# darskkaa/NTIRE-2026-Light-Field-Image-Super-Resolution-Challenge---Track-2-Efficiency

Hardware: AMD Instinct MI355X
Metric: 5x5 x4-SR LF patches/sec (32^2->128^2), DistgSSR inference (higher is better)
Workload: dtype f32 (EPI branch stage 1 / 2 and fuse.0: fp32 operands as three exact bf16 terms on the bf16 MFMA pipe, six products, fp32 accumulation -- error against fp64 not above the fp32-MFMA kernels', tests/test_gpu_b3_accuracy.py; 3x3 convs, angular branch, init, head: fp32 MFMA)

## Files before the change

### include/lfsr_hip.h

```cpp
#ifndef LFSR_HIP_H
#define LFSR_HIP_H

#include <stddef.h>
#include <stdint.h>

#ifdef __cplusplus
extern "C" {
#endif

#define LFSR_OK 0
#define LFSR_E_ARG (-1)
#define LFSR_E_WS (-2)

const char* lfsr_version(void);


int lfsr_sai2macpi(const void* in, void* out, int B, int C, int A, int h, int w, int elem_bytes, void* stream);
int lfsr_macpi2sai(const void* in, void* out, int B, int C, int A, int h, int w, int elem_bytes, void* stream);
int lfsr_pixel_shuffle2d(const void* in, void* out, int B, int C, int r, int H, int W, int elem_bytes, void* stream);
int lfsr_pixel_shuffle1d(const void* in, void* out, int B, int C, int f, int H, int W, int elem_bytes, void* stream);
int lfsr_image_extend(const void* in, void* out, int N, int h, int w, int top, int bottom, int left, int right,
                      int elem_bytes, void* stream);
int lfsr_lf_divide(const void* in, void* out, int A, int h0, int w0, int P, int S, int elem_bytes,
                   int* num_u, int* num_v, void* stream);
// ... 24 lines not shown
int lfsr_angconv_fwd(const float* x, int x_stride, int x_choff, const float* w1_packed, const float* w2_packed,
                     float* tmp, float* y, int y_stride, int y_choff, int B, int A, int h, int w, float slope, void* stream);

int lfsr_epiconv_fwd(const float* x, int x_stride, int x_choff, const float* w1_packed, const float* w2_packed,
                     float* tmp, float* y, int y_stride, int y_choff, int B, int A, int h, int w, int vertical,
                     float slope, void* stream);

int lfsr_epiconv_hv_fwd(const float* x, int x_stride, int x_choff, const float* w1_packed, const float* w2_packed,
                        float* tmp, float* y, int y_stride, int choff_h, int choff_v, int B, int A, int h, int w,
                        float slope, void* stream);

int lfsr_distg_branch_tail_fwd(const float* x, int x_stride, int x_choff, const float* spa, int spa_stride, int spa_choff,
                               const float* w_ang0, const float* w_ang2, const float* w_epi0, const float* w_epi2, const float* w_fuse0,
                               float* t_a, float* t_h, float* t_v, float* y, int y_stride, int y_choff, int B, int A, int h, int w, float slope,
                               void* stream);

int lfsr_initconv_fwd(const float* x, const float* w, float* y, int y_stride, int y_choff, int B, int A, int h, int wd,
                      void* stream);

int lfsr_fold_head(const float* w0, const float* b0, const float* w2, float* wf, float* bf, int C, int s, void* stream);
int lfsr_upsample_head_fwd(const float* f, int f_stride, int f_choff, const float* wf, const float* bf,
                           const float* x_lr, float* out, int B, int A, int h, int w, int s, void* stream);

typedef struct lfsr_distgssr lfsr_distgssr;

int lfsr_distgssr_create(lfsr_distgssr** ctx, int A, int scale, int n_group, int n_block, int channels);
void lfsr_distgssr_destroy(lfsr_distgssr* ctx);
size_t lfsr_distgssr_packed_bytes(const lfsr_distgssr* ctx);
int lfsr_distgssr_set_packed(lfsr_distgssr* ctx, void* packed, size_t bytes);
int lfsr_distgssr_load_param(lfsr_distgssr* ctx, const char* key, const float* data, size_t numel, void* stream);
// ... 181 lines not shown
```

### ntire-2026-light-field-image-super-resolution-challenge---track-2-efficiency_amd/capi.py

```python
import ctypes as C
import os

import torch

_HERE = os.path.dirname(os.path.abspath(__file__))
LIB_PATH = os.environ.get("LFSR_HIP_LIB") or os.path.join(_HERE, "liblfsr_hip.so")

c_p = C.c_void_p
c_i = C.c_int
c_f = C.c_float
c_sz = C.c_size_t

SIGNATURES = {
    "lfsr_version": (C.c_char_p, []),
    "lfsr_sai2macpi": (c_i, [c_p, c_p, c_i, c_i, c_i, c_i, c_i, c_i, c_p]),
    "lfsr_macpi2sai": (c_i, [c_p, c_p, c_i, c_i, c_i, c_i, c_i, c_i, c_p]),
    "lfsr_pixel_shuffle2d": (c_i, [c_p, c_p, c_i, c_i, c_i, c_i, c_i, c_i, c_p]),
    "lfsr_pixel_shuffle1d": (c_i, [c_p, c_p, c_i, c_i, c_i, c_i, c_i, c_i, c_p]),
    "lfsr_image_extend": (c_i, [c_p, c_p, c_i, c_i, c_i, c_i, c_i, c_i, c_i, c_i, c_p]),
    "lfsr_lf_divide": (c_i, [c_p, c_p, c_i, c_i, c_i, c_i, c_i, c_i, C.POINTER(c_i), C.POINTER(c_i), c_p]),
    "lfsr_lf_integrate": (c_i, [c_p, c_p, c_i, c_i, c_i, c_i, c_i, c_i, c_i, c_i, c_p]),
    "lfsr_lf_crop_tiles": (c_i, [c_p, c_p, c_i, c_i, c_i, c_i, c_i, c_p]),
    "lfsr_lf_place_tiles": (c_i, [c_p, c_p, c_i, c_i, c_i, c_i, c_i, c_i, c_i, c_i, c_i, c_p]),
    "lfsr_nchw_to_vcl": (c_i, [c_p, c_p, c_i, c_i, c_i, c_i, c_i, c_i, c_i, c_i, c_p]),
    "lfsr_vcl_to_nchw": (c_i, [c_p, c_i, c_i, c_p, c_i, c_i, c_i, c_i, c_i, c_i, c_p]),
    "lfsr_pack_conv_weight": (c_i, [c_p, c_p, c_i, c_i, c_i, c_i, c_i, c_p]),
    "lfsr_packed_weight_floats": (c_sz, [c_i, c_i, c_i]),
    "lfsr_conv3x3_fwd": (c_i, [c_p, c_i, c_i, c_p, c_p, c_i, c_i, c_p, c_i, c_i, c_p, c_i, c_i, c_i, c_i, c_i, c_f, c_p]),
    "lfsr_pointwise_fwd": (c_i, [c_p, c_i, c_i, c_i, c_p, c_p, c_p, c_i, c_i, c_i, c_i, c_f, c_p]),
    "lfsr_angconv_fwd": (c_i, [c_p, c_i, c_i, c_p, c_p, c_p, c_p, c_i, c_i, c_i, c_i, c_i, c_i, c_f, c_p]),
    "lfsr_epiconv_fwd": (c_i, [c_p, c_i, c_i, c_p, c_p, c_p, c_p, c_i, c_i, c_i, c_i, c_i, c_i, c_i, c_f, c_p]),
    "lfsr_epiconv_hv_fwd": (c_i, [c_p, c_i, c_i, c_p, c_p, c_p, c_p, c_i, c_i, c_i, c_i, c_i, c_i, c_i, c_f, c_p]),
    "lfsr_distg_branch_tail_fwd": (c_i, [c_p, c_i, c_i, c_p, c_i, c_i, c_p, c_p, c_p, c_p, c_p, c_p, c_p, c_p, c_p, c_i, c_i, c_i, c_i, c_i, c_i, c_f, c_p]),
    "lfsr_initconv_fwd": (c_i, [c_p, c_p, c_p, c_i, c_i, c_i, c_i, c_i, c_i, c_p]),
    "lfsr_fold_head": (c_i, [c_p, c_p, c_p, c_p, c_p, c_i, c_i, c_p]),
    "lfsr_upsample_head_fwd": (c_i, [c_p, c_i, c_i, c_p, c_p, c_p, c_p, c_i, c_i, c_i, c_i, c_i, c_p]),
    "lfsr_distgssr_begin_batched_load": (c_i, [c_p]),
    "lfsr_distgssr_forward_taps": (c_i, [c_p, c_p, c_p, c_i, c_i, c_i, c_p, c_sz, C.POINTER(c_p), c_p]),
    "lfsr_layernorm_fwd": (c_i, [c_p, c_i, c_i, c_p, c_i, C.c_longlong, C.c_longlong, c_p, c_p, c_p, c_i, c_i, C.c_longlong, c_i, c_f, c_p]),
    "lfsr_conv3x3_n_fwd": (c_i, [c_p, c_i, c_i, c_p, c_p, c_i, c_i, c_i, c_i, c_i, c_i, c_f, c_p]),
    "lfsr_lft_position_fwd": (c_i, [c_p, c_p, c_i, c_i, c_i, c_i, c_p]),
    "lfsr_view_metrics": (c_i, [c_p, c_p, c_p, c_p, c_i, c_i, c_i, c_i, c_p]),
    "lfsr_mask_views": (c_i, [c_p, c_p, c_p, c_f, c_i, c_i, c_i, c_i, c_i, c_p]),
    "lfsr_mask_views_fill": (c_i, [c_p, c_p, c_p, c_p, c_i, c_i, c_i, c_i, c_i, c_p]),
    "lfsr_linear_fwd": (c_i, [c_p, c_i, c_i, c_i, c_p, c_p, c_p, c_i, c_i, c_p, c_i, c_i, C.c_longlong, c_i, c_f, c_p]),
    "lfsr_ycbcr2rgb_views": (c_i, [c_p, c_p, c_p, c_i, c_i, c_i, C.POINTER(C.c_double), C.POINTER(C.c_double), c_p]),
    "lfsr_ffn_fwd": (c_i, [c_p, c_i, c_i, c_p, c_p, c_p, c_i, c_i, c_p, c_i, c_i, C.c_longlong, c_i, c_i, c_i, c_f, c_p]),
# ... 537 lines not shown
    return out


def distg_branch_tail(x, spa, w_ang0, w_ang2, w_epi0, w_epi2, w_fuse0, B, A, h, w, slope):
    lib = load()
    y = torch.empty((x.shape[0], 64), dtype=torch.float32, device=x.device)
    t_a = torch.empty((B * h * w, 16), dtype=torch.float32, device=x.device)
    t_h = torch.empty((B * A * h * w, 32), dtype=torch.float32, device=x.device)
    t_v = torch.empty((B * A * h * w, 32), dtype=torch.float32, device=x.device)
    check(lib.lfsr_distg_branch_tail_fwd(dev_ptr(x), x.shape[1], 0, dev_ptr(spa), spa.shape[1], 0, dev_ptr(w_ang0), dev_ptr(w_ang2), dev_ptr(w_epi0),
                                         dev_ptr(w_epi2), dev_ptr(w_fuse0), dev_ptr(t_a), dev_ptr(t_h), dev_ptr(t_v), dev_ptr(y), 64, 0, B, A, h, w, slope,
                                         stream_ptr()), "distg_branch_tail_fwd")
    return y, t_a, t_h, t_v


def initconv(x, w, A):
    lib = load()
    B, _, Hh, Ww = x.shape
    h, wd = Hh // A, Ww // A
    out = torch.empty((B * A * A * h * wd, 64), dtype=torch.float32, device=x.device)
    check(lib.lfsr_initconv_fwd(dev_ptr(x), dev_ptr(w), dev_ptr(out), 64, 0, B, A, h, wd, stream_ptr()), "initconv_fwd")
    return out


def upsample_head(f, w0, b0, w2, x_lr, A, s):
    lib = load()
    B, _, Hh, Ww = x_lr.shape
    h, w = Hh // A, Ww // A
    wf = torch.empty(s * s * 64, dtype=torch.float32, device=f.device)
    bf = torch.empty(s * s, dtype=torch.float32, device=f.device)
# ... 105 lines not shown
```

### ntire-2026-light-field-image-super-resolution-challenge---track-2-efficiency_amd/csrc/distg_tail.hip

```cpp
#include "lfsr_internal.h"

namespace {

typedef float f32x4t __attribute__((ext_vector_type(4)));
typedef unsigned u32x4t __attribute__((ext_vector_type(4)));

constexpr int DT_WAVES = 8;
constexpr int DT_FPLANE = 64 * 160;
constexpr int DT_FBYTES = 3 * DT_FPLANE * 2;
constexpr int DT_ESLOTS = 3 * 4 * 160;
constexpr int DT_EBYTES = DT_ESLOTS * 16;
constexpr int DT_AFLOATS = 25 * 16 * 16;
constexpr int DT_ABYTES = DT_AFLOATS * 4;
constexpr int DT_CROW = 84;
constexpr int DT_CBYTES = DT_WAVES * 16 * DT_CROW * 4;
constexpr int DT_SMEM = DT_FBYTES + DT_EBYTES + DT_ABYTES + DT_CBYTES;

struct DistgTailArgs {
  const float* S; int s_stride; int s_choff; int s_bytes;
  const float* TA; int ta_bytes;
  const float* TH; const float* TV; int te_bytes;
  const float* WA2;
  const uint4* WE2p;
  const float* WF;
// ... 229 lines not shown
  if (grid > cus[dev]) grid = cus[dev];
  hipLaunchKernelGGL(k_distg_tail, dim3((unsigned)grid), dim3(DT_WAVES * 64), DT_SMEM, st, p);
  LFSR_CHECK_LAUNCH();
  return LFSR_OK;
}

bool lfsr_distg_tail_ok(int A, int h, int w, const float* x, int x_stride, int x_choff, const float* t_h, const float* t_v) {
  if (A != 5 || h <= 0 || w <= 0 || h > 32 || w > 32 || !lfsr_ang_fused_ok(A) || !lfsr_epi_use_b3()) return false;
  const char* rsel = lfsr_sel("LFSR_ROWGEMM");
  const char* asel = lfsr_sel("LFSR_ANG");
  if ((rsel && (rsel[0] == 'f' || rsel[0] == '1')) || lfsr_sel("LFSR_NO_ROWGEMM") || (asel && asel[0] == 'g')) return false;
  if ((x_stride | x_choff) & 3 || x_stride < x_choff + 64 || (((uintptr_t)x | (uintptr_t)t_h | (uintptr_t)t_v) & 15)) return false;
  return true;
}

extern "C" int lfsr_distg_branch_tail_fwd(const float* x, int x_stride, int x_choff, const float* spa, int spa_stride, int spa_choff,
                                          const float* w_ang0, const float* w_ang2, const float* w_epi0, const float* w_epi2, const float* w_fuse0,
                                          float* t_a, float* t_h, float* t_v, float* y, int y_stride, int y_choff, int B, int A, int h, int w, float slope,
                                          void* stream) {
  LfsrOpTimer op_t("distg_tail", B, h * w, lfsr_stream(stream));
  if (!x || !spa || !w_ang0 || !w_ang2 || !w_epi0 || !w_epi2 || !w_fuse0 || !t_a || !t_h || !t_v || !y || B <= 0) return LFSR_E_ARG;
  if (!lfsr_distg_tail_ok(A, h, w, x, x_stride, x_choff, t_h, t_v)) return LFSR_E_ARG;
  if ((spa_stride | spa_choff | y_stride | y_choff) & 3 || spa_stride < spa_choff + 64 || y_stride < y_choff + 64) return LFSR_E_ARG;
  if (((uintptr_t)spa | (uintptr_t)t_a | (uintptr_t)w_ang2 | (uintptr_t)w_epi0 | (uintptr_t)w_epi2 | (uintptr_t)w_fuse0 | (uintptr_t)y) & 15) return LFSR_E_ARG;
  if (!(slope >= 0.f && slope <= 1.f)) return LFSR_E_ARG;
  const long long npix = (long long)B * A * A * h * w;
  if (npix * x_stride * 4 >= (1LL << 31) || npix * spa_stride * 4 >= (1LL << 31) || npix * y_stride * 4 >= (1LL << 31)) return LFSR_E_ARG;
  hipStream_t st = lfsr_stream(stream);
  int rc = lfsr_ang_fused_launch(x, x_stride, x_choff, w_ang0, nullptr, t_a, nullptr, 0, 0, B, A, h, w, slope, st);
  if (!rc) rc = lfsr_epi_b3_launch(x, x_stride, x_choff, w_epi0 + 25 * 32 * 64 + LFSR_EPI_WINO_FLOATS, nullptr, nullptr, 0, 0, 0, t_h, t_v, B, A, h, w, 3, slope, st);
  if (!rc) rc = lfsr_distg_tail_launch(spa, spa_stride, spa_choff, t_a, t_h, t_v, w_ang2, w_epi2 + 160 * 32, w_fuse0, y, y_stride, y_choff, B, A, h, w, slope, st);
  return rc;
}
```

### ntire-2026-light-field-image-super-resolution-challenge---track-2-efficiency_amd/csrc/distgssr.cpp

```cpp
#include <cstring>
#include <map>
#include <string>
#include <vector>

#include "param_table.h"

struct lfsr_distgssr : LfsrModel {
  int G = 0, NB = 0, C = 0;
  struct Transposed { int kind; size_t off; };
  std::map<std::string, Transposed> tr;
  size_t off_wf = 0, off_bf = 0;
  bool batch_mode = false;
  std::vector<LfsrPackDesc> d_gen, d_c3, d_epi, d_epib, uploaded;
  LfsrPackDesc* table_dev = nullptr;
  size_t table_cap = 0;
  hipStream_t side = nullptr;
  hipEvent_t ev_fork = nullptr, ev_join = nullptr, ev_a = nullptr, ev_b = nullptr;
  bool profiling = false;
  struct Ev { int cls; hipEvent_t a, b; };
  bool profile_all = true;
  int sample_stride = 1;
  long long sample_ctr = 0;
  std::vector<Ev> evs;
  std::vector<hipEvent_t> free_evs;
// ... 238 lines not shown
  };

  float* F0 = pool[0];
  PROF(4, lfsr_initconv_fwd(x, c->w("init_conv.weight"), F0, 64, 0, B, A, h, w, stream));
  LFSR_RC(tap(0, F0, 64, 64));
  const float* cur = F0;
  for (int g = 0; g < c->G; ++g) {
    const float* gin = cur;
    for (int b = 0; b < c->NB; ++b) {
      std::string p = "disentg.Group." + std::to_string(g) + ".Block." + std::to_string(b) + ".";
      float* o = pick(F0, gin, cur);
      PROF(0, conv(cur, p + "SpaConv.0.weight", T, 64, 0, nullptr, L));
      if (tail_ok && !(taps && taps[4] && g == 0 && b == 0)) {
        PROF(0, conv(T, p + "SpaConv.2.weight", o, 64, 0, nullptr, L));
        hipStream_t st = lfsr_stream(stream);
        PROF(1, lfsr_ang_fused_launch(cur, 64, 0, c->w(p + "AngConv.0.weight"), nullptr, A16, nullptr, 0, 0, B, A, h, w, L, st));
        PROF(2, lfsr_epi_b3_launch(cur, 64, 0, c->w(p + "EPIConv.0.weight") + 25 * 32 * 64 + LFSR_EPI_WINO_FLOATS, nullptr, nullptr, 0, 0, 0, E32, EV32,
                                   B, A, h, w, 3, L, st));
        PROF(3, lfsr_distg_tail_launch(o, 64, 0, A16, E32, EV32, c->w(p + "AngConv.2.weight"), c->w(p + "EPIConv.2.weight") + 160 * 32,
                                       c->w(p + "fuse.0.weight"), T, 64, 0, B, A, h, w, L, st));
        PROF(0, conv(T, p + "fuse.2.weight", o, 64, 0, cur, 1.0f));
        cur = o;
        if (g == 0 && b == 0) LFSR_RC(tap(1, cur, 64, 64));
        continue;
      }
      PROF(0, conv(T, p + "SpaConv.2.weight", CAT, 144, 0, nullptr, L));
      PROF(1, lfsr_angconv_fwd(cur, 64, 0, c->w(p + "AngConv.0.weight"), c->w(p + "AngConv.2.weight"), A16, CAT, 144, 64, B, A, h, w, L, stream));
      PROF(2, lfsr_epiconv_hv_fwd(cur, 64, 0, c->w(p + "EPIConv.0.weight"), c->w(p + "EPIConv.2.weight"), E32, CAT, 144, 80, 112, B, A, h, w, L, stream));
      if (g == 0 && b == 0) LFSR_RC(tap(4, CAT, 144, 144));
      PROF(3, lfsr_pointwise_fwd(CAT, 144, 0, 144, c->w(p + "fuse.0.weight"), nullptr, T, 64, 0, nimg * h * w, 64, L, stream));
      PROF(0, conv(T, p + "fuse.2.weight", o, 64, 0, cur, 1.0f));
      cur = o;
      if (g == 0 && b == 0) LFSR_RC(tap(1, cur, 64, 64));
// ... 291 lines not shown
```

### ntire-2026-light-field-image-super-resolution-challenge---track-2-efficiency_amd/csrc/epi_b3.hip

```cpp
#include <stdlib.h>

#include "lfsr_internal.h"

#ifndef EB_VAR
#define EB_VAR 0
#endif
#ifndef EB_ABL
#define EB_ABL 0
#endif

namespace {

typedef float f32x4e __attribute__((ext_vector_type(4)));
typedef unsigned u32x4e __attribute__((ext_vector_type(4)));

constexpr int EB_LINES = 8;
constexpr int EB_STAGE_SLOTS = 5 * 3 * 4 * 32;
constexpr int EB_STAGE_BYTES = EB_STAGE_SLOTS * 16;
constexpr int EB_W2_SLOTS = 3 * 4 * 160;
constexpr int EB_W2_BYTES = EB_W2_SLOTS * 16;
constexpr int EB_SMEM = 4 * EB_STAGE_BYTES + EB_W2_BYTES;
constexpr int EB_SMEM1 = 4 * EB_STAGE_BYTES;

struct EpiB3Args {
  const float* X; int x_stride; int x_choff; int x_bytes;
  const uint4* W1p;
  const uint4* W2p;
  float* Y; int y_stride; int choffH; int choffV; int y_bytes;
  float* TH; float* TV;
  int B, H, W;
  int tilesH, tilesV;
  int tpiH, tpiV;
  float slope;
};

__device__ __forceinline__ unsigned eb_hi_pair(unsigned hi_src, unsigned lo_src) { return __builtin_amdgcn_perm(hi_src, lo_src, 0x07060302u); }
__device__ __forceinline__ float eb_residual(float a) { return a - __uint_as_float(__float_as_uint(a) & 0xffff0000u); }

__device__ __forceinline__ void eb_split8(const f32x4e lo, const f32x4e hi, u32x4e& p0, u32x4e& p1, u32x4e& p2) {
  const float a[8] = {lo.x, lo.y, lo.z, lo.w, hi.x, hi.y, hi.z, hi.w};
#pragma unroll
  for (int j = 0; j < 4; ++j) { unsigned t0, t1, t2; lfsr_split_pair(a[2 * j], a[2 * j + 1], t0, t1, t2); p0[j] = t0; p1[j] = t1; p2[j] = t2; }
}

__device__ __forceinline__ void eb_mfma(f32x4e& c, const u32x4e a, const u32x4e b) {
  asm volatile("v_mfma_f32_16x16x32_bf16 %0, %1, %2, %0" : "+v"(c) : "v"(a), "v"(b));
}

// ... 12 lines not shown
  return __builtin_bit_cast(float, __builtin_amdgcn_update_dpp(0, __builtin_bit_cast(int, v), CTRL, 0xf, 0xf, true));
}
template <int D>
__device__ __forceinline__ void eb_shift_add(f32x4e (&t)[2], const f32x4e (&z)[2]) {
  constexpr int SAME = D > 0 ? 0x100 + D : 0x110 - D;
  constexpr int WRAP = D > 0 ? 0x110 + (16 - D) : 0x100 + (16 + D);
#pragma unroll
  for (int r = 0; r < 4; ++r) {
    t[0][r] += eb_dpp0<SAME>(z[0][r]);
    t[1][r] += eb_dpp0<SAME>(z[1][r]);
    if (D > 0) t[0][r] += eb_dpp0<WRAP>(z[1][r]);
    else t[1][r] += eb_dpp0<WRAP>(z[0][r]);
  }
}

template <bool S2>
__global__ __launch_bounds__(512) void k_epi_b3(EpiB3Args p) {
  extern __shared__ __attribute__((aligned(16))) unsigned char smem_raw[];
  unsigned char* const sW = smem_raw;
  unsigned char* const sW2 = smem_raw + 4 * EB_STAGE_BYTES;
  constexpr int A = 5;
  constexpr int EOOB = (int)0x80000000u;
  const int tid = threadIdx.x, lane = tid & 63, wave = tid >> 6;
  const int l15 = lane & 15, g = lane >> 4;
  const int phase = __builtin_amdgcn_readfirstlane(wave >> 2);
  const int HW = p.H * p.W;
  const int ngroups = p.tilesH + p.tilesV;
  const int nb = (int)gridDim.x;
  const int vb = (nb & 7) ? (int)blockIdx.x : ((int)blockIdx.x & 7) * (nb >> 3) + ((int)blockIdx.x >> 3);

  const __amdgpu_buffer_rsrc_t rsX = __builtin_amdgcn_make_buffer_rsrc(const_cast<float*>(p.X), 0, p.x_bytes, 0x00020000);
  const __amdgpu_buffer_rsrc_t rsY = __builtin_amdgcn_make_buffer_rsrc(p.Y, 0, p.y_bytes, 0x00020000);

  struct Line { int vert, base, len, vstride, pstride, choff; long long rowbase; int rowstep; };
  const int nfr = ngroups / nb, nfull = nfr * nb, rem = ngroups - nfull;
  const int fsub = rem == 0 ? 1 : (rem * 4 <= nb ? 4 : rem * 2 <= nb ? 2 : 1);
  const int nunits = nfr + (vb < rem * fsub ? 1 : 0);
  auto line_of = [&](int it) -> Line {
// ... 31 lines not shown

  f32x4e rawA[2][2], rawB[2][2];
  u32x4e pA0[2], pA1[2], pA2[2], pB0[2], pB1[2], pB2[2];
  auto load_x = [&](const Line& L, int j, f32x4e (&xr)[2][2]) {
    const int vv = j >> 1, ks = j & 1;
    const int soff = (vv * L.vstride * p.x_stride + 32 * ks) * 4;
#pragma unroll
    for (int nt = 0; nt < 2; ++nt) {
      const int s = 16 * nt + l15;
      const int off = (L.base >= 0 && s < L.len) ? ((L.base + s * L.pstride) * p.x_stride + p.x_choff + 8 * g) * 4 : EOOB;
      xr[nt][0] = __builtin_bit_cast(f32x4e, __builtin_amdgcn_raw_buffer_load_b128(rsX, off, soff, 0));
      xr[nt][1] = __builtin_bit_cast(f32x4e, __builtin_amdgcn_raw_buffer_load_b128(rsX, off == EOOB ? EOOB : off + 16, soff, 0));
    }
  };
  uint4 wr[4];
  auto load_w = [&](int half_idx) {
    const uint4* src = p.W1p + half_idx * EB_STAGE_SLOTS;
#pragma unroll
    for (int i = 0; i < 4; ++i) {
      const int idx = tid + 512 * i;
      wr[i] = idx < EB_STAGE_SLOTS ? src[idx] : make_uint4(0u, 0u, 0u, 0u);
    }
  };
  auto store_w = [&](int buf, int ks) {
    uint4* dst = reinterpret_cast<uint4*>(sW + (buf * 2 + ks) * EB_STAGE_BYTES);
#pragma unroll
    for (int i = 0; i < 4; ++i) {
      const int idx = tid + 512 * i;
      if (idx < EB_STAGE_SLOTS) dst[idx] = wr[i];
    }
  };

  int it = 0;
  if (nunits == 0) return;
  Line L = line_of(0);
  load_x(L, 0, rawA);
  load_x(L, 1, rawB);
  load_w(0);
  if (S2) {
    uint4 w2r[4];
#pragma unroll
    for (int i = 0; i < 4; ++i) { const int idx = tid + 512 * i; w2r[i] = idx < EB_W2_SLOTS ? p.W2p[idx] : make_uint4(0u, 0u, 0u, 0u); }
#pragma unroll
    for (int i = 0; i < 4; ++i) { const int idx = tid + 512 * i; if (idx < EB_W2_SLOTS) reinterpret_cast<uint4*>(sW2)[idx] = w2r[i]; }
  }
  store_w(0, 0);
  load_w(1);
  store_w(0, 1);
#pragma unroll
  for (int nt = 0; nt < 2; ++nt) eb_split8(rawA[nt][0], rawA[nt][1], pA0[nt], pA1[nt], pA2[nt]);
  __syncthreads();
  int cur = 0;
  const int aoff = (g * 32 + l15) * 16;
  const unsigned char* const w2b = sW2 + (g * 160 + l15) * 16;

  for (;;) {
    const bool more = it + 1 < nunits;
    const Line Ln = line_of(it + 1);
    f32x4e acc[5][2][2];
#pragma unroll
    for (int dx = 0; dx < 5; ++dx)
#pragma unroll
      for (int mt = 0; mt < 2; ++mt) { acc[dx][mt][0] = f32x4e{0.f, 0.f, 0.f, 0.f}; acc[dx][mt][1] = acc[dx][mt][0]; }
#pragma unroll
    for (int dx = 0; dx < 5; ++dx) asm volatile("s_nop 1" : "+v"(acc[dx][0][0]), "+v"(acc[dx][0][1]), "+v"(acc[dx][1][0]), "+v"(acc[dx][1][1]));

    auto step = [&](int j, u32x4e (&u0)[2], u32x4e (&u1)[2], u32x4e (&u2)[2], f32x4e (&rs)[2][2], u32x4e (&d0)[2], u32x4e (&d1)[2], u32x4e (&d2)[2],
                    f32x4e (&rd)[2][2]) {
      const int vv = j >> 1, ks = j & 1;
      if (!(EB_ABL & 8)) {
        if (j + 2 < 10) load_x(L, j + 2, rd);
        else load_x(Ln, j + 2 - 10, rd);
      }
      if (!(EB_ABL & 4)) load_w(2 * (vv + 1 < A ? vv + 1 : 0) + ks);
      asm volatile("s_nop 4" : "+v"(u0[0]), "+v"(u1[0]), "+v"(u2[0]), "+v"(u0[1]), "+v"(u1[1]), "+v"(u2[1]));
      const unsigned char* wb = sW + (cur * 2 + ks) * EB_STAGE_BYTES + aoff;
      u32x4e af[2][3];
      auto load_a = [&](int c, u32x4e (&a)[3]) {
        const int dx = c >> 1, mt = c & 1;
#pragma unroll
        for (int pl = 0; pl < 3; ++pl) a[pl] = *reinterpret_cast<const u32x4e*>(wb + ((dx * 3 + pl) * 128 + 16 * mt) * 16);
      };
      load_a(0, af[0]);
#pragma unroll
      for (int c = 0; c < 10; ++c) {
        const int dx = c >> 1, mt = c & 1;
        if (c + 1 < 10 && !(EB_ABL & 2)) load_a(c + 1, af[(c + 1) & 1]);
        constexpr int ABL2 = (EB_ABL & 2) ? 0 : 1;
        eb_six2(acc[dx][mt][0], acc[dx][mt][1], af[(c & 1) * ABL2][0], af[(c & 1) * ABL2][1], af[(c & 1) * ABL2][2], u0[0], u1[0], u2[0], u0[1], u1[1], u2[1]);
        if (!(EB_ABL & 1) && c == ((phase && !(EB_VAR & 4)) ? 5 : 0)) {
          asm volatile("" : "+v"(rs[0][0]), "+v"(rs[0][1]), "+v"(rs[1][0]), "+v"(rs[1][1]));
#pragma unroll
          for (int nt = 0; nt < 2; ++nt) eb_split8(rs[nt][0], rs[nt][1], d0[nt], d1[nt], d2[nt]);
          asm volatile("" : "+v"(d0[0]), "+v"(d1[0]), "+v"(d2[0]), "+v"(d0[1]), "+v"(d1[1]), "+v"(d2[1]));
        }
      }
      if (!(EB_ABL & 4)) store_w(cur ^ 1, ks);
      if (ks) { if (!(EB_ABL & 32)) __syncthreads(); cur ^= 1; }
    };
#pragma unroll 1
    for (int jj = 0; jj < 10; jj += 2) {
      step(jj, pA0, pA1, pA2, rawB, pB0, pB1, pB2, rawA);
      step(jj + 1, pB0, pB1, pB2, rawA, pA0, pA1, pA2, rawB);
    }

#pragma unroll
    for (int dx = 0; dx < 5; ++dx)
      asm volatile("s_nop 15\n\ts_nop 15" : "+v"(acc[dx][0][0]), "+v"(acc[dx][0][1]), "+v"(acc[dx][1][0]), "+v"(acc[dx][1][1]));
    if (EB_ABL & 16) {
      f32x4e sacc = acc[0][0][0];
// ... 127 lines not shown

int lfsr_pack_epi_b3(const float* direct_packed, float* out, int kind, hipStream_t st) {
  if (!direct_packed || !out || (kind != 0 && kind != 1) || ((uintptr_t)out & 15)) return LFSR_E_ARG;
  hipLaunchKernelGGL(k_pack_epi_b3, dim3(kind == 0 ? 25 : 3), dim3(256), 0, st, direct_packed, reinterpret_cast<uint4*>(out), kind);
  LFSR_CHECK_LAUNCH();
  return LFSR_OK;
}

int lfsr_pack_epi_b3_batch(const LfsrPackDesc* table_dev, int n, hipStream_t st) {
  if (!table_dev || n <= 0) return n == 0 ? LFSR_OK : LFSR_E_ARG;
  hipLaunchKernelGGL(k_pack_epi_b3_batch, dim3(25, (unsigned)n), dim3(256), 0, st, table_dev);
  LFSR_CHECK_LAUNCH();
  return LFSR_OK;
}

int lfsr_epi_b3_launch(const float* x, int x_stride, int x_choff, const float* w1_planes, const float* w2_planes, float* y, int y_stride,
                       int choffH, int choffV, float* t_h, float* t_v, int B, int A, int h, int w, int which, float slope, hipStream_t st) {
  if (A != 5 || h > 32 || w > 32 || h <= 0 || w <= 0 || B <= 0) return LFSR_E_ARG;
  if (!y && (which != 3 || !t_h || !t_v)) return LFSR_E_ARG;
  if ((x_stride | x_choff | y_stride | choffH | choffV) & 3) return LFSR_E_ARG;
  if (((uintptr_t)x | (uintptr_t)y | (uintptr_t)w1_planes | (uintptr_t)w2_planes | (uintptr_t)t_h | (uintptr_t)t_v) & 15) return LFSR_E_ARG;
  if ((long long)B * A * A * h * w * x_stride * 4 >= (1LL << 31) || (y && (long long)B * A * A * h * w * y_stride * 4 >= (1LL << 31))) return LFSR_E_ARG;
  if (!(slope >= 0.f && slope <= 1.f)) return LFSR_E_ARG;
  static std::atomic<bool> attr_set[64];
  static std::atomic<int> cus[64];
  int dev = 0;
  if (hipGetDevice(&dev) != hipSuccess || dev < 0 || dev >= 64) return LFSR_E_ARG;
  if (!attr_set[dev]) {
    hipError_t e = hipFuncSetAttribute(reinterpret_cast<const void*>(k_epi_b3<true>), hipFuncAttributeMaxDynamicSharedMemorySize, EB_SMEM);
    if (e == hipSuccess) e = hipFuncSetAttribute(reinterpret_cast<const void*>(k_epi_b3<false>), hipFuncAttributeMaxDynamicSharedMemorySize, EB_SMEM1);
    if (e != hipSuccess) return LFSR_HIP_ERR(e);
    int v = 0;
    cus[dev] = (hipDeviceGetAttribute(&v, hipDeviceAttributeMultiprocessorCount, dev) == hipSuccess && v > 0) ? v : 256;
    attr_set[dev] = true;
  }
  EpiB3Args p{};
  p.X = x; p.x_stride = x_stride; p.x_choff = x_choff; p.x_bytes = (int)((long long)B * A * A * h * w * x_stride * 4);
  p.W1p = reinterpret_cast<const uint4*>(w1_planes); p.W2p = reinterpret_cast<const uint4*>(w2_planes);
  p.Y = y; p.y_stride = y_stride; p.choffH = choffH; p.choffV = choffV; p.TH = t_h; p.TV = t_v;
  p.y_bytes = y ? (int)((long long)B * A * A * h * w * y_stride * 4) : 0;
  p.B = B; p.H = h; p.W = w; p.slope = slope;
  p.tilesH = (which & 1) ? (B * A * h + EB_LINES - 1) / EB_LINES : 0;
  p.tilesV = (which & 2) ? (B * A * w + EB_LINES - 1) / EB_LINES : 0;
  const int ngroups = p.tilesH + p.tilesV;
  if (ngroups <= 0) return LFSR_E_ARG;
  if (which == 3 && (A * h) % EB_LINES == 0 && (A * w) % EB_LINES == 0) { p.tpiH = A * h / EB_LINES; p.tpiV = A * w / EB_LINES; }
  int grid = cus[dev];
  if (grid > ngroups) grid = ngroups;
  if (y) hipLaunchKernelGGL(k_epi_b3<true>, dim3((unsigned)grid), dim3(512), EB_SMEM, st, p);
  else hipLaunchKernelGGL(k_epi_b3<false>, dim3((unsigned)grid), dim3(512), EB_SMEM1, st, p);
  LFSR_CHECK_LAUNCH();
  return LFSR_OK;
}
```

### ntire-2026-light-field-image-super-resolution-challenge---track-2-efficiency_amd/csrc/lfsr_internal.h

```cpp
#pragma once
#include <functional>
#include <string>

#include "lfsr_common.h"

enum { LFSR_IN_SAME = 0, LFSR_IN_CONV3 = 1, LFSR_IN_ANG = 2, LFSR_IN_EPIH = 3, LFSR_IN_EPIV = 4,
       LFSR_IN_CHK_H = 5, LFSR_IN_CHK_V = 6, LFSR_IN_LINE_H = 7, LFSR_IN_LINE_V = 8 };
enum { LFSR_OUT_SAME = 0, LFSR_OUT_VIEWS = 1, LFSR_OUT_EPIH = 2, LFSR_OUT_EPIV = 3 };

#if defined(__HIPCC__)
#ifndef LFSR_SPLIT_DOT2
#define LFSR_SPLIT_DOT2 1
#endif
__device__ __forceinline__ void lfsr_split_pair(float a0, float a1, unsigned& p0, unsigned& p1, unsigned& p2) {
  typedef __bf16 lfsr_bf16x2 __attribute__((ext_vector_type(2)));
  p0 = __builtin_amdgcn_perm(__float_as_uint(a1), __float_as_uint(a0), 0x07060302u);
#if LFSR_SPLIT_DOT2
  unsigned klo, khi;
  asm("s_mov_b32 %0, 0xbf80" : "=s"(klo));
  asm("s_mov_b32 %0, 0xbf800000" : "=s"(khi));
  const float r0 = __builtin_amdgcn_fdot2_f32_bf16(__builtin_bit_cast(lfsr_bf16x2, p0), __builtin_bit_cast(lfsr_bf16x2, klo), a0, false);
  const float r1 = __builtin_amdgcn_fdot2_f32_bf16(__builtin_bit_cast(lfsr_bf16x2, p0), __builtin_bit_cast(lfsr_bf16x2, khi), a1, false);
  p1 = __builtin_amdgcn_perm(__float_as_uint(r1), __float_as_uint(r0), 0x07060302u);
  const float q0 = __builtin_amdgcn_fdot2_f32_bf16(__builtin_bit_cast(lfsr_bf16x2, p1), __builtin_bit_cast(lfsr_bf16x2, klo), r0, false);
// ... 63 lines not shown
int lfsr_pack_wino_m(const float* direct_packed, float* out, int mask, hipStream_t st);
int lfsr_pack_conv_weight_m(const float* w, float* packed, int O, int C, int taps, int perm, int ch, int mask, void* stream);
int lfsr_pack_weight_T_m(const float* w, float* out, int O, int C, int T, int flip, int mask, hipStream_t st);
int lfsr_pack_wino4(const float* direct_packed, float* out, hipStream_t st);
bool lfsr_ang_fused_ok(int A);
int lfsr_ang_fused_launch(const float* x, int x_stride, int x_choff, const float* w1_packed, const float* w2_packed, float* t, float* y,
                          int y_stride, int y_choff, int B, int A, int h, int w, float slope, hipStream_t st);
#define LFSR_EPI_WINO_FLOATS (5 * 6 * 32 * 64)
#define LFSR_EPI_B3_W1_FLOATS (25 * 32 * 64 * 3 / 2)
#define LFSR_EPI_B3_W2_FLOATS (160 * 32 * 3 / 2)
bool lfsr_epi_use_b3();
int lfsr_pack_epi_b3(const float* direct_packed, float* out, int kind, hipStream_t st);
int lfsr_pack_epi_b3_batch(const LfsrPackDesc* table_dev, int n, hipStream_t st);
int lfsr_epi_b3_launch(const float* x, int x_stride, int x_choff, const float* w1_planes, const float* w2_planes, float* y, int y_stride,
                       int choffH, int choffV, float* t_h, float* t_v, int B, int A, int h, int w, int which, float slope, hipStream_t st);
int lfsr_pack_epi_wino(const float* w1_direct_packed, float* out, hipStream_t st);
bool lfsr_distg_tail_ok(int A, int h, int w, const float* x, int x_stride, int x_choff, const float* t_h, const float* t_v);
int lfsr_distg_tail_launch(const float* spa, int spa_stride, int spa_choff, const float* t_a, const float* t_h, const float* t_v, const float* wa2_packed,
                           const float* we2_planes, const float* wf_packed, float* y, int y_stride, int y_choff, int B, int A, int h, int w, float slope,
                           hipStream_t st);
bool lfsr_epi_fused_ok(int A, int h, int w);
int lfsr_epi_fused_launch(const float* x, int x_stride, int x_choff, const float* w1_packed, const float* w2_packed, float* y, int y_stride,
                          int choffH, int choffV, float* t_h, float* t_v, int B, int A, int h, int w, int which, float slope, hipStream_t st);

extern "C" int lfsr_epiconv_gather(const float* x, int x_stride, int x_choff, const float* w1_packed, const float* w2_packed,
                        float* tmp, float* y, int y_stride, int y_choff, int B, int A, int h, int w, int vertical, float slope, hipStream_t st);

struct LfsrGemm {
  int in_mode, out_mode, cin;
  const float* X; int x_stride, x_choff;
// ... 162 lines not shown
```

Measured before the change: 2097.

## Fuse angular-branch stage-1 conv into the EPI b3 stage-1 kernel

Runs the angular conv (AngConv.0) inside the EPI bf16x3 stage-1 kernel instead of as a separate launch. Some waves' weight-staging slots are repurposed to stream angular weight slices into extra LDS, and each wave interleaves fp32 MFMA angular work with the EPI pipeline, writing t_a directly. This removes one kernel launch and a second pass over the input features. The cost is extra LDS, more register pressure and interleaved work that could slow the EPI critical path. It only applies when the geometry check passes, and an env var can disable it.

```diff
diff --git a/include/lfsr_hip.h b/include/lfsr_hip.h
--- a/include/lfsr_hip.h
+++ b/include/lfsr_hip.h
@@ -62,6 +62,10 @@
                                const float* w_ang0, const float* w_ang2, const float* w_epi0, const float* w_epi2, const float* w_fuse0,
                                float* t_a, float* t_h, float* t_v, float* y, int y_stride, int y_choff, int B, int A, int h, int w, float slope,
                                void* stream);
+
+int lfsr_distg_stage1_fwd(const float* x, int x_stride, int x_choff, const float* w_ang0, const float* w_epi0, float* t_a, float* t_h, float* t_v,
+                          int B, int A, int h, int w, float slope, void* stream);
+int lfsr_distg_stage1_covers(int B, int A, int h, int w);
 
 int lfsr_initconv_fwd(const float* x, const float* w, float* y, int y_stride, int y_choff, int B, int A, int h, int wd,
                       void* stream);
diff --git a/ntire-2026-light-field-image-super-resolution-challenge---track-2-efficiency_amd/capi.py b/ntire-2026-light-field-image-super-resolution-challenge---track-2-efficiency_amd/capi.py
--- a/ntire-2026-light-field-image-super-resolution-challenge---track-2-efficiency_amd/capi.py
+++ b/ntire-2026-light-field-image-super-resolution-challenge---track-2-efficiency_amd/capi.py
@@ -31,6 +31,8 @@
     "lfsr_angconv_fwd": (c_i, [c_p, c_i, c_i, c_p, c_p, c_p, c_p, c_i, c_i, c_i, c_i, c_i, c_i, c_f, c_p]),
     "lfsr_epiconv_fwd": (c_i, [c_p, c_i, c_i, c_p, c_p, c_p, c_p, c_i, c_i, c_i, c_i, c_i, c_i, c_i, c_f, c_p]),
     "lfsr_epiconv_hv_fwd": (c_i, [c_p, c_i, c_i, c_p, c_p, c_p, c_p, c_i, c_i, c_i, c_i, c_i, c_i, c_i, c_f, c_p]),
+    "lfsr_distg_stage1_covers": (c_i, [c_i, c_i, c_i, c_i]),
+    "lfsr_distg_stage1_fwd": (c_i, [c_p, c_i, c_i, c_p, c_p, c_p, c_p, c_p, c_i, c_i, c_i, c_i, c_f, c_p]),
     "lfsr_distg_branch_tail_fwd": (c_i, [c_p, c_i, c_i, c_p, c_i, c_i, c_p, c_p, c_p, c_p, c_p, c_p, c_p, c_p, c_p, c_i, c_i, c_i, c_i, c_i, c_i, c_f, c_p]),
     "lfsr_initconv_fwd": (c_i, [c_p, c_p, c_p, c_i, c_i, c_i, c_i, c_i, c_i, c_p]),
     "lfsr_fold_head": (c_i, [c_p, c_p, c_p, c_p, c_p, c_i, c_i, c_p]),
@@ -598,6 +600,20 @@
     return y, t_a, t_h, t_v
 
 
+def distg_stage1_covers(B, A, h, w):
+    return bool(load().lfsr_distg_stage1_covers(B, A, h, w))
+
+
+def distg_stage1(x, w_ang0, w_epi0, B, A, h, w, slope, x_choff=0):
+    lib = load()
+    t_a = torch.empty((B * h * w, 16), dtype=torch.float32, device=x.device)
+    t_h = torch.empty((B * A * h * w, 32), dtype=torch.float32, device=x.device)
+    t_v = torch.empty((B * A * h * w, 32), dtype=torch.float32, device=x.device)
+    check(lib.lfsr_distg_stage1_fwd(dev_ptr(x), x.shape[1], x_choff, dev_ptr(w_ang0), dev_ptr(w_epi0), dev_ptr(t_a), dev_ptr(t_h), dev_ptr(t_v),
+                                    B, A, h, w, slope, stream_ptr()), "distg_stage1_fwd")
+    return t_a, t_h, t_v
+
+
 def initconv(x, w, A):
     lib = load()
     B, _, Hh, Ww = x.shape
diff --git a/ntire-2026-light-field-image-super-resolution-challenge---track-2-efficiency_amd/csrc/distg_tail.hip b/ntire-2026-light-field-image-super-resolution-challenge---track-2-efficiency_amd/csrc/distg_tail.hip
--- a/ntire-2026-light-field-image-super-resolution-challenge---track-2-efficiency_amd/csrc/distg_tail.hip
+++ b/ntire-2026-light-field-image-super-resolution-challenge---track-2-efficiency_amd/csrc/distg_tail.hip
@@ -267,6 +267,29 @@
   return true;
 }
 
+int lfsr_distg_stage1(const float* x, int x_stride, int x_choff, const float* w_ang0_packed, const float* w_epi0_planes, float* t_a, float* t_h, float* t_v,
+                      int B, int A, int h, int w, float slope, hipStream_t st) {
+  const char* sel = lfsr_sel("LFSR_DISTG_STAGE1");
+  if (!(sel && sel[0] == '0') && lfsr_distg_stage1_ok(B, A, h, w))
+    return lfsr_distg_stage1_launch(x, x_stride, x_choff, w_ang0_packed, w_epi0_planes, t_a, t_h, t_v, B, A, h, w, slope, st);
+  int rc = lfsr_ang_fused_launch(x, x_stride, x_choff, w_ang0_packed, nullptr, t_a, nullptr, 0, 0, B, A, h, w, slope, st);
+  if (!rc) rc = lfsr_epi_b3_launch(x, x_stride, x_choff, w_epi0_planes, nullptr, nullptr, 0, 0, 0, t_h, t_v, B, A, h, w, 3, slope, st);
+  return rc;
+}
+
+extern "C" int lfsr_distg_stage1_covers(int B, int A, int h, int w) { return lfsr_distg_stage1_ok(B, A, h, w) ? 1 : 0; }
+
+extern "C" int lfsr_distg_stage1_fwd(const float* x, int x_stride, int x_choff, const float* w_ang0, const float* w_epi0, float* t_a, float* t_h, float* t_v,
+                                     int B, int A, int h, int w, float slope, void* stream) {
+  LfsrOpTimer op_t("distg_stage1", B, h * w, lfsr_stream(stream));
+  if (!x || !w_ang0 || !w_epi0 || !t_a || !t_h || !t_v || B <= 0) return LFSR_E_ARG;
+  if (!lfsr_distg_tail_ok(A, h, w, x, x_stride, x_choff, t_h, t_v)) return LFSR_E_ARG;
+  if (((uintptr_t)t_a | (uintptr_t)w_ang0 | (uintptr_t)w_epi0) & 15) return LFSR_E_ARG;
+  if (!(slope >= 0.f && slope <= 1.f)) return LFSR_E_ARG;
+  if ((long long)B * A * A * h * w * x_stride * 4 >= (1LL << 31)) return LFSR_E_ARG;
+  return lfsr_distg_stage1(x, x_stride, x_choff, w_ang0, w_epi0 + 25 * 32 * 64 + LFSR_EPI_WINO_FLOATS, t_a, t_h, t_v, B, A, h, w, slope, lfsr_stream(stream));
+}
+
 extern "C" int lfsr_distg_branch_tail_fwd(const float* x, int x_stride, int x_choff, const float* spa, int spa_stride, int spa_choff,
                                           const float* w_ang0, const float* w_ang2, const float* w_epi0, const float* w_epi2, const float* w_fuse0,
                                           float* t_a, float* t_h, float* t_v, float* y, int y_stride, int y_choff, int B, int A, int h, int w, float slope,
@@ -280,8 +303,7 @@
   const long long npix = (long long)B * A * A * h * w;
   if (npix * x_stride * 4 >= (1LL << 31) || npix * spa_stride * 4 >= (1LL << 31) || npix * y_stride * 4 >= (1LL << 31)) return LFSR_E_ARG;
   hipStream_t st = lfsr_stream(stream);
-  int rc = lfsr_ang_fused_launch(x, x_stride, x_choff, w_ang0, nullptr, t_a, nullptr, 0, 0, B, A, h, w, slope, st);
-  if (!rc) rc = lfsr_epi_b3_launch(x, x_stride, x_choff, w_epi0 + 25 * 32 * 64 + LFSR_EPI_WINO_FLOATS, nullptr, nullptr, 0, 0, 0, t_h, t_v, B, A, h, w, 3, slope, st);
+  int rc = lfsr_distg_stage1(x, x_stride, x_choff, w_ang0, w_epi0 + 25 * 32 * 64 + LFSR_EPI_WINO_FLOATS, t_a, t_h, t_v, B, A, h, w, slope, st);
   if (!rc) rc = lfsr_distg_tail_launch(spa, spa_stride, spa_choff, t_a, t_h, t_v, w_ang2, w_epi2 + 160 * 32, w_fuse0, y, y_stride, y_choff, B, A, h, w, slope, st);
   return rc;
 }
diff --git a/ntire-2026-light-field-image-super-resolution-challenge---track-2-efficiency_amd/csrc/distgssr.cpp b/ntire-2026-light-field-image-super-resolution-challenge---track-2-efficiency_amd/csrc/distgssr.cpp
--- a/ntire-2026-light-field-image-super-resolution-challenge---track-2-efficiency_amd/csrc/distgssr.cpp
+++ b/ntire-2026-light-field-image-super-resolution-challenge---track-2-efficiency_amd/csrc/distgssr.cpp
@@ -276,9 +276,14 @@
       if (tail_ok && !(taps && taps[4] && g == 0 && b == 0)) {
         PROF(0, conv(T, p + "SpaConv.2.weight", o, 64, 0, nullptr, L));
         hipStream_t st = lfsr_stream(stream);
-        PROF(1, lfsr_ang_fused_launch(cur, 64, 0, c->w(p + "AngConv.0.weight"), nullptr, A16, nullptr, 0, 0, B, A, h, w, L, st));
-        PROF(2, lfsr_epi_b3_launch(cur, 64, 0, c->w(p + "EPIConv.0.weight") + 25 * 32 * 64 + LFSR_EPI_WINO_FLOATS, nullptr, nullptr, 0, 0, 0, E32, EV32,
-                                   B, A, h, w, 3, L, st));
+        if (c->profiling && c->profile_all) {
+          PROF(1, lfsr_ang_fused_launch(cur, 64, 0, c->w(p + "AngConv.0.weight"), nullptr, A16, nullptr, 0, 0, B, A, h, w, L, st));
+          PROF(2, lfsr_epi_b3_launch(cur, 64, 0, c->w(p + "EPIConv.0.weight") + 25 * 32 * 64 + LFSR_EPI_WINO_FLOATS, nullptr, nullptr, 0, 0, 0, E32, EV32,
+                                     B, A, h, w, 3, L, st));
+        } else {
+          PROF(2, lfsr_distg_stage1(cur, 64, 0, c->w(p + "AngConv.0.weight"), c->w(p + "EPIConv.0.weight") + 25 * 32 * 64 + LFSR_EPI_WINO_FLOATS, A16, E32, EV32,
+                                    B, A, h, w, L, st));
+        }
         PROF(3, lfsr_distg_tail_launch(o, 64, 0, A16, E32, EV32, c->w(p + "AngConv.2.weight"), c->w(p + "EPIConv.2.weight") + 160 * 32,
                                        c->w(p + "fuse.0.weight"), T, 64, 0, B, A, h, w, L, st));
         PROF(0, conv(T, p + "fuse.2.weight", o, 64, 0, cur, 1.0f));
diff --git a/ntire-2026-light-field-image-super-resolution-challenge---track-2-efficiency_amd/csrc/epi_b3.hip b/ntire-2026-light-field-image-super-resolution-challenge---track-2-efficiency_amd/csrc/epi_b3.hip
--- a/ntire-2026-light-field-image-super-resolution-challenge---track-2-efficiency_amd/csrc/epi_b3.hip
+++ b/ntire-2026-light-field-image-super-resolution-challenge---track-2-efficiency_amd/csrc/epi_b3.hip
@@ -21,6 +21,9 @@
 constexpr int EB_W2_BYTES = EB_W2_SLOTS * 16;
 constexpr int EB_SMEM = 4 * EB_STAGE_BYTES + EB_W2_BYTES;
 constexpr int EB_SMEM1 = 4 * EB_STAGE_BYTES;
+constexpr int EA_ROW = 68, EA_TROW = 20;
+constexpr int EA_SLICE_FLOATS = 16 * EA_ROW;
+constexpr int EB_SMEMA = EB_SMEM1 + (2 * EA_SLICE_FLOATS + EB_LINES * 16 * EA_TROW + 512 * 4) * 4;
 
 struct EpiB3Args {
   const float* X; int x_stride; int x_choff; int x_bytes;
@@ -32,6 +35,9 @@
   int tilesH, tilesV;
   int tpiH, tpiV;
   float slope;
+  const float* WA;
+  float* TA;
+  int unitsA;
 };
 
 __device__ __forceinline__ unsigned eb_hi_pair(unsigned hi_src, unsigned lo_src) { return __builtin_amdgcn_perm(hi_src, lo_src, 0x07060302u); }
@@ -74,14 +80,16 @@
   }
 }
 
-template <bool S2>
+template <bool S2, bool ANG = false>
 __global__ __launch_bounds__(512) void k_epi_b3(EpiB3Args p) {
+  static_assert(!(S2 && ANG), "ANG rides on the stage-1-only kernel");
   extern __shared__ __attribute__((aligned(16))) unsigned char smem_raw[];
   unsigned char* const sW = smem_raw;
   unsigned char* const sW2 = smem_raw + 4 * EB_STAGE_BYTES;
   constexpr int A = 5;
   constexpr int EOOB = (int)0x80000000u;
-  const int tid = threadIdx.x, lane = tid & 63, wave = tid >> 6;
+  const int tid = threadIdx.x, lane = tid & 63;
+  const int wave = ANG ? __builtin_amdgcn_readfirstlane(tid >> 6) : tid >> 6;
   const int l15 = lane & 15, g = lane >> 4;
   const int phase = __builtin_amdgcn_readfirstlane(wave >> 2);
   const int HW = p.H * p.W;
@@ -143,12 +151,19 @@
     }
   };
   uint4 wr[4];
-  auto load_w = [&](int half_idx) {
+  float* const sA = reinterpret_cast<float*>(smem_raw + EB_SMEM1);
+  const bool astage = wave >= (EB_STAGE_SLOTS - 3 * 512) / 64;
+  const int aslot = tid & 127;
+  const __amdgpu_buffer_rsrc_t rsWA = __builtin_amdgcn_make_buffer_rsrc(const_cast<float*>(p.WA), 0, ANG ? A * A * 32 * 64 * 4 : 0, 0x00020000);
+  auto load_w = [&](int half_idx, int atap) {
     const uint4* src = p.W1p + half_idx * EB_STAGE_SLOTS;
 #pragma unroll
     for (int i = 0; i < 4; ++i) {
       const int idx = tid + 512 * i;
-      wr[i] = idx < EB_STAGE_SLOTS ? src[idx] : make_uint4(0u, 0u, 0u, 0u);
+      if (ANG && i == 3) {
+        if (!astage) wr[i] = src[idx];
+        else wr[i] = __builtin_bit_cast(uint4, __builtin_amdgcn_raw_buffer_load_b128(rsWA, ((aslot >> 4) * 64 + (aslot & 15) * 4) * 4, ((atap * 32 + 8 * (half_idx & 1)) * 64) * 4, 0));
+      } else wr[i] = idx < EB_STAGE_SLOTS ? src[idx] : make_uint4(0u, 0u, 0u, 0u);
     }
   };
   auto store_w = [&](int buf, int ks) {
@@ -156,8 +171,25 @@
 #pragma unroll
     for (int i = 0; i < 4; ++i) {
       const int idx = tid + 512 * i;
-      if (idx < EB_STAGE_SLOTS) dst[idx] = wr[i];
-    }
+      if (ANG && i == 3) {
+        if (!astage) dst[idx] = wr[i];
+        else *reinterpret_cast<uint4*>(sA + buf * EA_SLICE_FLOATS + ((aslot >> 4) + 8 * ks) * EA_ROW + (aslot & 15) * 4) = wr[i];
+      } else if (idx < EB_STAGE_SLOTS) dst[idx] = wr[i];
+    }
+  };
+  f32x4e fragA[2];
+  f32x4e* const saccA = reinterpret_cast<f32x4e*>(sA + 2 * EA_SLICE_FLOATS + EB_LINES * 16 * EA_TROW) + tid;
+  int offA = EOOB, kA = 0, tapA = 0;
+  auto ang_unit = [&](int k) {
+    const int u = (k * EB_LINES + wave) * nb + vb, m = 16 * u + l15;
+    const bool ok = k < nfr / A && u < p.unitsA && m < p.B * HW;
+    const int mb = ok ? m / HW : 0, myx = m - mb * HW;
+    offA = ok ? ((mb * A * A * HW + myx) * p.x_stride + p.x_choff + 4 * g) * 4 : EOOB;
+  };
+  auto load_frag = [&](int tap, int hf) {
+#pragma unroll
+    for (int jj = 0; jj < 2; ++jj)
+      fragA[jj] = __builtin_bit_cast(f32x4e, __builtin_amdgcn_raw_buffer_load_b128(rsX, offA, (tap * HW * p.x_stride + 16 * (2 * hf + jj)) * 4, 0));
   };
 
   int it = 0;
@@ -165,7 +197,8 @@
   Line L = line_of(0);
   load_x(L, 0, rawA);
   load_x(L, 1, rawB);
-  load_w(0);
+  if (ANG) { ang_unit(0); load_frag(0, 0); *saccA = f32x4e{0.f, 0.f, 0.f, 0.f}; }
+  load_w(0, 0);
   if (S2) {
     uint4 w2r[4];
 #pragma unroll
@@ -174,7 +207,7 @@
     for (int i = 0; i < 4; ++i) { const int idx = tid + 512 * i; if (idx < EB_W2_SLOTS) reinterpret_cast<uint4*>(sW2)[idx] = w2r[i]; }
   }
   store_w(0, 0);
-  load_w(1);
+  load_w(1, 0);
   store_w(0, 1);
 #pragma unroll
   for (int nt = 0; nt < 2; ++nt) eb_split8(rawA[nt][0], rawA[nt][1], pA0[nt], pA1[nt], pA2[nt]);
@@ -201,7 +234,7 @@
         if (j + 2 < 10) load_x(L, j + 2, rd);
         else load_x(Ln, j + 2 - 10, rd);
       }
-      if (!(EB_ABL & 4)) load_w(2 * (vv + 1 < A ? vv + 1 : 0) + ks);
+      if (!(EB_ABL & 4)) load_w(2 * (vv + 1 < A ? vv + 1 : 0) + ks, tapA + 1 < A * A ? tapA + 1 : 0);
       asm volatile("s_nop 4" : "+v"(u0[0]), "+v"(u1[0]), "+v"(u2[0]), "+v"(u0[1]), "+v"(u1[1]), "+v"(u2[1]));
       const unsigned char* wb = sW + (cur * 2 + ks) * EB_STAGE_BYTES + aoff;
       u32x4e af[2][3];
@@ -223,6 +256,37 @@
           for (int nt = 0; nt < 2; ++nt) eb_split8(rs[nt][0], rs[nt][1], d0[nt], d1[nt], d2[nt]);
           asm volatile("" : "+v"(d0[0]), "+v"(d1[0]), "+v"(d2[0]), "+v"(d0[1]), "+v"(d1[1]), "+v"(d2[1]));
         }
+      }
+      if (ANG) {
+        int bo = l15 * EA_ROW + 4 * g;
+        asm volatile("" : "+v"(fragA[0]), "+v"(fragA[1]), "+v"(bo));
+        const float* bt = sA + cur * EA_SLICE_FLOATS + bo + 32 * ks;
+        f32x4e accA = *saccA;
+#pragma unroll
+        for (int jj = 0; jj < 2; ++jj) {
+          const f32x4e b = *reinterpret_cast<const f32x4e*>(bt + 16 * jj), a = fragA[jj];
+          accA = __builtin_amdgcn_mfma_f32_16x16x4f32(a.x, b.x, accA, 0, 0, 0);
+          accA = __builtin_amdgcn_mfma_f32_16x16x4f32(a.y, b.y, accA, 0, 0, 0);
+          accA = __builtin_amdgcn_mfma_f32_16x16x4f32(a.z, b.z, accA, 0, 0, 0);
+          accA = __builtin_amdgcn_mfma_f32_16x16x4f32(a.w, b.w, accA, 0, 0, 0);
+        }
+        if (ks) {
+          if (tapA == A * A - 1) {
+            float* tt = sA + 2 * EA_SLICE_FLOATS + wave * 16 * EA_TROW;
+#pragma unroll
+            for (int r = 0; r < 4; ++r) { const float v = accA[r]; tt[(4 * g + r) * EA_TROW + l15] = v >= 0.f ? v : v * p.slope; }
+            __builtin_amdgcn_wave_barrier();
+            const f32x4e row = *reinterpret_cast<const f32x4e*>(tt + l15 * EA_TROW + 4 * g);
+            const int m = 16 * ((kA * EB_LINES + wave) * nb + vb) + l15;
+            if (offA != EOOB) *reinterpret_cast<f32x4e*>(p.TA + (long long)m * 16 + 4 * g) = row;
+            __builtin_amdgcn_wave_barrier();
+            accA = f32x4e{0.f, 0.f, 0.f, 0.f};
+            tapA = 0; ++kA;
+            ang_unit(kA);
+          } else ++tapA;
+          load_frag(tapA, 0);
+        } else load_frag(tapA, 1);
+        *saccA = accA;
       }
       if (!(EB_ABL & 4)) store_w(cur ^ 1, ks);
       if (ks) { if (!(EB_ABL & 32)) __syncthreads(); cur ^= 1; }
@@ -380,41 +444,86 @@
   return LFSR_OK;
 }
 
-int lfsr_epi_b3_launch(const float* x, int x_stride, int x_choff, const float* w1_planes, const float* w2_planes, float* y, int y_stride,
-                       int choffH, int choffV, float* t_h, float* t_v, int B, int A, int h, int w, int which, float slope, hipStream_t st) {
-  if (A != 5 || h > 32 || w > 32 || h <= 0 || w <= 0 || B <= 0) return LFSR_E_ARG;
-  if (!y && (which != 3 || !t_h || !t_v)) return LFSR_E_ARG;
-  if ((x_stride | x_choff | y_stride | choffH | choffV) & 3) return LFSR_E_ARG;
-  if (((uintptr_t)x | (uintptr_t)y | (uintptr_t)w1_planes | (uintptr_t)w2_planes | (uintptr_t)t_h | (uintptr_t)t_v) & 15) return LFSR_E_ARG;
-  if ((long long)B * A * A * h * w * x_stride * 4 >= (1LL << 31) || (y && (long long)B * A * A * h * w * y_stride * 4 >= (1LL << 31))) return LFSR_E_ARG;
-  if (!(slope >= 0.f && slope <= 1.f)) return LFSR_E_ARG;
+namespace {
+
+int eb_device_cus(hipError_t* err) {
   static std::atomic<bool> attr_set[64];
   static std::atomic<int> cus[64];
   int dev = 0;
-  if (hipGetDevice(&dev) != hipSuccess || dev < 0 || dev >= 64) return LFSR_E_ARG;
+  *err = hipSuccess;
+  if (hipGetDevice(&dev) != hipSuccess || dev < 0 || dev >= 64) return 0;
   if (!attr_set[dev]) {
     hipError_t e = hipFuncSetAttribute(reinterpret_cast<const void*>(k_epi_b3<true>), hipFuncAttributeMaxDynamicSharedMemorySize, EB_SMEM);
     if (e == hipSuccess) e = hipFuncSetAttribute(reinterpret_cast<const void*>(k_epi_b3<false>), hipFuncAttributeMaxDynamicSharedMemorySize, EB_SMEM1);
-    if (e != hipSuccess) return LFSR_HIP_ERR(e);
+    if (e == hipSuccess) e = hipFuncSetAttribute(reinterpret_cast<const void*>(k_epi_b3<false, true>), hipFuncAttributeMaxDynamicSharedMemorySize, EB_SMEMA);
+    if (e != hipSuccess) { *err = e; return 0; }
     int v = 0;
     cus[dev] = (hipDeviceGetAttribute(&v, hipDeviceAttributeMultiprocessorCount, dev) == hipSuccess && v > 0) ? v : 256;
     attr_set[dev] = true;
   }
+  return cus[dev];
+}
+
+struct EbGeom { int tilesH, tilesV, grid, upw; long long unitsA; };
+EbGeom eb_geom(int B, int A, int h, int w, int which, int cus) {
+  EbGeom q{};
+  q.tilesH = (which & 1) ? (B * A * h + EB_LINES - 1) / EB_LINES : 0;
+  q.tilesV = (which & 2) ? (B * A * w + EB_LINES - 1) / EB_LINES : 0;
+  const int ngroups = q.tilesH + q.tilesV;
+  q.grid = cus < ngroups ? cus : ngroups;
+  q.upw = q.grid > 0 ? ngroups / q.grid / A : 0;
+  q.unitsA = ((long long)B * h * w + 15) / 16;
+  return q;
+}
+
+int eb_launch(const float* x, int x_stride, int x_choff, const float* w1_planes, const float* w2_planes, float* y, int y_stride,
+              int choffH, int choffV, const float* w_ang, float* t_a, float* t_h, float* t_v, int B, int A, int h, int w, int which, float slope, hipStream_t st) {
+  if (A != 5 || h > 32 || w > 32 || h <= 0 || w <= 0 || B <= 0) return LFSR_E_ARG;
+  if (!y && (which != 3 || !t_h || !t_v)) return LFSR_E_ARG;
+  if ((x_stride | x_choff | y_stride | choffH | choffV) & 3) return LFSR_E_ARG;
+  if (((uintptr_t)x | (uintptr_t)y | (uintptr_t)w1_planes | (uintptr_t)w2_planes | (uintptr_t)t_h | (uintptr_t)t_v | (uintptr_t)w_ang | (uintptr_t)t_a) & 15) return LFSR_E_ARG;
+  if ((long long)B * A * A * h * w * x_stride * 4 >= (1LL << 31) || (y && (long long)B * A * A * h * w * y_stride * 4 >= (1LL << 31))) return LFSR_E_ARG;
+  if (!(slope >= 0.f && slope <= 1.f)) return LFSR_E_ARG;
+  hipError_t herr;
+  const int cus = eb_device_cus(&herr);
+  if (cus <= 0) return herr != hipSuccess ? LFSR_HIP_ERR(herr) : LFSR_E_ARG;
+  const EbGeom q = eb_geom(B, A, h, w, which, cus);
   EpiB3Args p{};
   p.X = x; p.x_stride = x_stride; p.x_choff = x_choff; p.x_bytes = (int)((long long)B * A * A * h * w * x_stride * 4);
   p.W1p = reinterpret_cast<const uint4*>(w1_planes); p.W2p = reinterpret_cast<const uint4*>(w2_planes);
   p.Y = y; p.y_stride = y_stride; p.choffH = choffH; p.choffV = choffV; p.TH = t_h; p.TV = t_v;
   p.y_bytes = y ? (int)((long long)B * A * A * h * w * y_stride * 4) : 0;
   p.B = B; p.H = h; p.W = w; p.slope = slope;
-  p.tilesH = (which & 1) ? (B * A * h + EB_LINES - 1) / EB_LINES : 0;
-  p.tilesV = (which & 2) ? (B * A * w + EB_LINES - 1) / EB_LINES : 0;
-  const int ngroups = p.tilesH + p.tilesV;
-  if (ngroups <= 0) return LFSR_E_ARG;
+  p.tilesH = q.tilesH; p.tilesV = q.tilesV;
+  p.WA = w_ang; p.TA = t_a; p.unitsA = (int)q.unitsA;
+  if (q.grid <= 0) return LFSR_E_ARG;
   if (which == 3 && (A * h) % EB_LINES == 0 && (A * w) % EB_LINES == 0) { p.tpiH = A * h / EB_LINES; p.tpiV = A * w / EB_LINES; }
-  int grid = cus[dev];
-  if (grid > ngroups) grid = ngroups;
+  const int grid = q.grid;
   if (y) hipLaunchKernelGGL(k_epi_b3<true>, dim3((unsigned)grid), dim3(512), EB_SMEM, st, p);
+  else if (t_a) hipLaunchKernelGGL((k_epi_b3<false, true>), dim3((unsigned)grid), dim3(512), EB_SMEMA, st, p);
   else hipLaunchKernelGGL(k_epi_b3<false>, dim3((unsigned)grid), dim3(512), EB_SMEM1, st, p);
   LFSR_CHECK_LAUNCH();
   return LFSR_OK;
 }
+
+}
+
+int lfsr_epi_b3_launch(const float* x, int x_stride, int x_choff, const float* w1_planes, const float* w2_planes, float* y, int y_stride,
+                       int choffH, int choffV, float* t_h, float* t_v, int B, int A, int h, int w, int which, float slope, hipStream_t st) {
+  return eb_launch(x, x_stride, x_choff, w1_planes, w2_planes, y, y_stride, choffH, choffV, nullptr, nullptr, t_h, t_v, B, A, h, w, which, slope, st);
+}
+
+bool lfsr_distg_stage1_ok(int B, int A, int h, int w) {
+  if (A != 5 || h > 32 || w > 32 || h <= 0 || w <= 0 || B <= 0 || B >= (1 << 20)) return false;
+  hipError_t e;
+  const int cus = eb_device_cus(&e);
+  if (cus <= 0) return false;
+  const EbGeom q = eb_geom(B, A, h, w, 3, cus);
+  return q.upw >= 1 && q.unitsA <= (long long)q.grid * EB_LINES * q.upw;
+}
+
+int lfsr_distg_stage1_launch(const float* x, int x_stride, int x_choff, const float* w_ang0_packed, const float* w_epi0_planes, float* t_a, float* t_h, float* t_v,
+                             int B, int A, int h, int w, float slope, hipStream_t st) {
+  if (!w_ang0_packed || !t_a || !t_h || !t_v || !lfsr_distg_stage1_ok(B, A, h, w)) return LFSR_E_ARG;
+  return eb_launch(x, x_stride, x_choff, w_epi0_planes, nullptr, nullptr, 0, 0, 0, w_ang0_packed, t_a, t_h, t_v, B, A, h, w, 3, slope, st);
+}
diff --git a/ntire-2026-light-field-image-super-resolution-challenge---track-2-efficiency_amd/csrc/lfsr_internal.h b/ntire-2026-light-field-image-super-resolution-challenge---track-2-efficiency_amd/csrc/lfsr_internal.h
--- a/ntire-2026-light-field-image-super-resolution-challenge---track-2-efficiency_amd/csrc/lfsr_internal.h
+++ b/ntire-2026-light-field-image-super-resolution-challenge---track-2-efficiency_amd/csrc/lfsr_internal.h
@@ -101,6 +101,11 @@
 int lfsr_pack_epi_b3_batch(const LfsrPackDesc* table_dev, int n, hipStream_t st);
 int lfsr_epi_b3_launch(const float* x, int x_stride, int x_choff, const float* w1_planes, const float* w2_planes, float* y, int y_stride,
                        int choffH, int choffV, float* t_h, float* t_v, int B, int A, int h, int w, int which, float slope, hipStream_t st);
+bool lfsr_distg_stage1_ok(int B, int A, int h, int w);
+int lfsr_distg_stage1_launch(const float* x, int x_stride, int x_choff, const float* w_ang0_packed, const float* w_epi0_planes, float* t_a, float* t_h, float* t_v,
+                             int B, int A, int h, int w, float slope, hipStream_t st);
+int lfsr_distg_stage1(const float* x, int x_stride, int x_choff, const float* w_ang0_packed, const float* w_epi0_planes, float* t_a, float* t_h, float* t_v,
+                      int B, int A, int h, int w, float slope, hipStream_t st);
 int lfsr_pack_epi_wino(const float* w1_direct_packed, float* out, hipStream_t st);
 bool lfsr_distg_tail_ok(int A, int h, int w, const float* x, int x_stride, int x_choff, const float* t_h, const float* t_v);
 int lfsr_distg_tail_launch(const float* spa, int spa_stride, int spa_choff, const float* t_a, const float* t_h, const float* t_v, const float* wa2_packed,
```

After: 2112, median of 6. No clear change (+0.7%).
